# hku-mars/GS-SDF

Hardware: NVIDIA H100
Metric: train_steps_per_s (higher is better)
Workload: dtype f32

## Files before the change

gs-sdf_b200/csrc/sdf_tc.cu:

```cuda
#include "sdf_grid.cuh"
#include "sdf_loss.cuh"

namespace gssdf {

constexpr int kFwdTcThreads = 256;
constexpr int kBwdTcThreads = 512;
constexpr int kLevels = 16;
static_assert(128 * kLevels == 4 * kBwdTcThreads, "encode batches assume 4 tasks per thread");
constexpr uint32_t kWImg = 24576;
constexpr uint32_t kGW = 3072;
constexpr uint32_t kGA = 2048;
constexpr uint32_t kGA0 = 1024;
constexpr uint32_t kGL = 1024;

__device__ __forceinline__ uint32_t off_act(int r, int k, int part) {
    return (uint32_t)((r >> 3) * kGA + part * 1024 + (k >> 3) * 128 + (r & 7) * 16 + (k & 7) * 2);
}
__device__ __forceinline__ uint32_t off_feat(int r, int k, int part) {
    return (uint32_t)((r >> 3) * kGA0 + part * 512 + (k >> 3) * 128 + (r & 7) * 16 + (k & 7) * 2);
}
__device__ __forceinline__ uint32_t off_lo(int r, int k) { return (uint32_t)((r >> 3) * kGL + (k >> 3) * 128 + (r & 7) * 16 + (k & 7) * 2); }
__device__ __host__ __forceinline__ uint32_t off_w(int o, int k, int part) {
    return (uint32_t)((o >> 3) * kGW + part * 1024 + (k >> 3) * 128 + (o & 7) * 16 + (k & 7) * 2);
}

__device__ __forceinline__ uint64_t make_desc(uint32_t saddr, uint32_t lbo, uint32_t sbo) {
    uint64_t d = 0;
    d |= (uint64_t)((saddr & 0x3FFFF) >> 4);
    d |= (uint64_t)(lbo >> 4) << 16;
    d |= (uint64_t)(sbo >> 4) << 32;
    return d;
}
__device__ __forceinline__ void wg_fence() { asm volatile("wgmma.fence.sync.aligned;" ::: "memory"); }
__device__ __forceinline__ void wg_commit() { asm volatile("wgmma.commit_group.sync.aligned;" ::: "memory"); }
__device__ __forceinline__ void wg_wait() { asm volatile("wgmma.wait_group.sync.aligned 0;" ::: "memory"); }
template <int R>
__device__ __forceinline__ void acc_fence(float (&d)[R]) {
#pragma unroll
    for (int i = 0; i < R; ++i) asm volatile("" : "+f"(d[i])::"memory");
}
template <int TA, int TB>
__device__ __forceinline__ void wgmma_bf16(float (&d)[16], uint64_t a, uint64_t b, uint32_t accumulate) {
    asm volatile(
        "{\n"
        ".reg .pred p;\n"
        "setp.ne.b32 p, %18, 0;\n"
        "wgmma.mma_async.sync.aligned.m64n32k16.f32.bf16.bf16 {%0, %1, %2, %3, %4, %5, %6, %7, %8, %9, %10, %11, %12, %13, %14, %15}, "
        "%16, %17, p, 1, 1, %19, %20;\n"
        "}\n"
        : "+f"(d[0]), "+f"(d[1]), "+f"(d[2]), "+f"(d[3]), "+f"(d[4]), "+f"(d[5]), "+f"(d[6]), "+f"(d[7]), "+f"(d[8]), "+f"(d[9]),
          "+f"(d[10]), "+f"(d[11]), "+f"(d[12]), "+f"(d[13]), "+f"(d[14]), "+f"(d[15])
        : "l"(a), "l"(b), "r"(accumulate), "n"(TA), "n"(TB)
        : "memory");
}
template <int TA, int TB>
__device__ __forceinline__ void wgmma_bf16(float (&d)[32], uint64_t a, uint64_t b, uint32_t accumulate) {
    asm volatile(
        "{\n"
        ".reg .pred p;\n"
        "setp.ne.b32 p, %34, 0;\n"
        "wgmma.mma_async.sync.aligned.m64n64k16.f32.bf16.bf16 {%0, %1, %2, %3, %4, %5, %6, %7, %8, %9, %10, %11, %12, %13, %14, %15, "
        "%16, %17, %18, %19, %20, %21, %22, %23, %24, %25, %26, %27, %28, %29, %30, %31}, %32, %33, p, 1, 1, %35, %36;\n"
        "}\n"
        : "+f"(d[0]), "+f"(d[1]), "+f"(d[2]), "+f"(d[3]), "+f"(d[4]), "+f"(d[5]), "+f"(d[6]), "+f"(d[7]), "+f"(d[8]), "+f"(d[9]),
          "+f"(d[10]), "+f"(d[11]), "+f"(d[12]), "+f"(d[13]), "+f"(d[14]), "+f"(d[15]), "+f"(d[16]), "+f"(d[17]), "+f"(d[18]),
          "+f"(d[19]), "+f"(d[20]), "+f"(d[21]), "+f"(d[22]), "+f"(d[23]), "+f"(d[24]), "+f"(d[25]), "+f"(d[26]), "+f"(d[27]),
          "+f"(d[28]), "+f"(d[29]), "+f"(d[30]), "+f"(d[31])
        : "l"(a), "l"(b), "r"(accumulate), "n"(TA), "n"(TB)
        : "memory");
}
__device__ __forceinline__ bool mbar_wait_bounded(uint64_t *bar, uint32_t parity) {
    for (int it = 0; it < (1 << 24); ++it) {
        uint32_t ok;
        asm volatile(
            "{\n"
            ".reg .pred p;\n"
            "mbarrier.try_wait.parity.shared::cta.b64 p, [%1], %2;\n"
            "selp.u32 %0, 1, 0, p;\n"
            "}\n"
            : "=r"(ok)
            : "r"(smem_u32(bar)), "r"(parity)
            : "memory");
        if (ok) return true;
    }
    return false;
}

__device__ __forceinline__ void split2(float x, __nv_bfloat16 &hi, __nv_bfloat16 &mid) {
    hi = __float2bfloat16_rn(x);
    mid = __float2bfloat16_rn(x - __bfloat162float(hi));
}
__device__ __forceinline__ void split3(float x, __nv_bfloat16 &hi, __nv_bfloat16 &mid, __nv_bfloat16 &lo) {
    hi = __float2bfloat16_rn(x);
    const float r1 = x - __bfloat162float(hi);
    mid = __float2bfloat16_rn(r1);
    lo = __float2bfloat16_rn(r1 - __bfloat162float(mid));
}
__device__ __forceinline__ void store8(unsigned char *buf, unsigned char *lo_buf, int r, int k0, const float *x) {
    __nv_bfloat16 hi[8], mid[8], lo[8];
#pragma unroll
    for (int e = 0; e < 8; ++e) split3(x[e], hi[e], mid[e], lo[e]);
    *reinterpret_cast<uint4 *>(buf + off_act(r, k0, 0)) = *reinterpret_cast<uint4 *>(hi);
    *reinterpret_cast<uint4 *>(buf + off_act(r, k0, 1)) = *reinterpret_cast<uint4 *>(mid);
    if (lo_buf) *reinterpret_cast<uint4 *>(lo_buf + off_lo(r, k0)) = *reinterpret_cast<uint4 *>(lo);
}
__device__ __forceinline__ void load8_hi(const unsigned char *buf, int r, int k0, float *x) {
    const uint4 h = *reinterpret_cast<const uint4 *>(buf + off_act(r, k0, 0));
    const __nv_bfloat16 *hp = reinterpret_cast<const __nv_bfloat16 *>(&h);
#pragma unroll
    for (int e = 0; e < 8; ++e) x[e] = __bfloat162float(hp[e]);
}
__device__ __forceinline__ void load8_sum(const unsigned char *buf, int r, int k0, float *x) {
    const uint4 h = *reinterpret_cast<const uint4 *>(buf + off_act(r, k0, 0));
    const uint4 m = *reinterpret_cast<const uint4 *>(buf + off_act(r, k0, 1));
    const __nv_bfloat16 *hp = reinterpret_cast<const __nv_bfloat16 *>(&h), *mp = reinterpret_cast<const __nv_bfloat16 *>(&m);
#pragma unroll
    for (int e = 0; e < 8; ++e) x[e] = __bfloat162float(hp[e]) + __bfloat162float(mp[e]);
}
__device__ __forceinline__ void store2(unsigned char *buf, unsigned char *lo_buf, int r, int k0, float x0, float x1) {
    __nv_bfloat16 h0, m0, l0, h1, m1, l1;
    split3(x0, h0, m0, l0);
    split3(x1, h1, m1, l1);
    *reinterpret_cast<__nv_bfloat162 *>(buf + off_act(r, k0, 0)) = __halves2bfloat162(h0, h1);
    *reinterpret_cast<__nv_bfloat162 *>(buf + off_act(r, k0, 1)) = __halves2bfloat162(m0, m1);
    if (lo_buf) *reinterpret_cast<__nv_bfloat162 *>(lo_buf + off_lo(r, k0)) = __halves2bfloat162(l0, l1);
}
__device__ __forceinline__ float2 load2_hi(const unsigned char *buf, int r, int k0) {
    return __bfloat1622float2(*reinterpret_cast<const __nv_bfloat162 *>(buf + off_act(r, k0, 0)));
}
__device__ __forceinline__ float quad_sum(float v) {
    v += __shfl_xor_sync(0xffffffffu, v, 1);
    return v + __shfl_xor_sync(0xffffffffu, v, 2);
}
__device__ __forceinline__ float colsum16(float c[16], int lane) {
#pragma unroll
    for (int s = 8; s >= 1; s >>= 1) {
        const bool up = lane & s;
#pragma unroll
        for (int k = 0; k < s; ++k) {
            const float send = up ? c[k] : c[k + s], keep = up ? c[k + s] : c[k];
            c[k] = keep + __shfl_xor_sync(0xffffffffu, send, s);
        }
    }
    return c[0] + __shfl_xor_sync(0xffffffffu, c[0], 16);
}

template <bool FEAT, bool THREE, int R>
__device__ __forceinline__ void issue_layer(float (&d)[R], uint32_t a_base, uint32_t lo_base, uint32_t w_base) {
    constexpr uint32_t ga = FEAT ? kGA0 : kGA, am = FEAT ? 512u : 1024u;
    wg_fence();
#pragma unroll
    for (int ks = 0; ks < (FEAT ? kFeat : 64) / 16; ++ks) {
        const uint32_t ko = ks * 256;
        const uint64_t ah = make_desc(a_base + ko, 128, ga), amd = make_desc(a_base + am + ko, 128, ga);
        const uint64_t wh = make_desc(w_base + ko, 128, kGW), wm = make_desc(w_base + 1024 + ko, 128, kGW);
        wgmma_bf16<0, 0>(d, ah, wh, ks > 0 ? 1u : 0u);
        wgmma_bf16<0, 0>(d, ah, wm, 1);
        wgmma_bf16<0, 0>(d, amd, wh, 1);
        wgmma_bf16<0, 0>(d, amd, wm, 1);
        if constexpr (THREE) {
            wgmma_bf16<0, 0>(d, ah, make_desc(w_base + 2048 + ko, 128, kGW), 1);
            if constexpr (!FEAT) wgmma_bf16<0, 0>(d, make_desc(lo_base + ko, 128, kGL), wh, 1);
        }
    }
    wg_commit();
}
template <bool THREE = true, int R>
__device__ __forceinline__ void issue_forward_layer(float (&d)[R], int l, uint32_t a_base, uint32_t lo_base, uint32_t w_base) {
    if (l == 0) issue_layer<true, THREE>(d, a_base, lo_base, w_base);
    else issue_layer<false, THREE>(d, a_base, lo_base, w_base);
}

__global__ void __launch_bounds__(256) mlp_pack_kernel(const float *__restrict__ mlp, unsigned char *__restrict__ packed, int n_layers) {
    const int l = blockIdx.x;
    const int K = l == 0 ? kFeat : 64;
    const float *W = mlp;
    for (int q = 0; q < l; ++q) W += (size_t)64 * (q == 0 ? kFeat : 64) + 64;
    unsigned char *img = packed + (size_t)l * kWImg;
    for (int e = threadIdx.x; e < 64 * 64; e += blockDim.x) {
        const int o = e >> 6, k = e & 63;
        __nv_bfloat16 hi, mid, lo;
        split3(k < K ? __ldg(W + (size_t)o * K + k) : 0.f, hi, mid, lo);
        *reinterpret_cast<__nv_bfloat16 *>(img + off_w(o, k, 0)) = hi;
        *reinterpret_cast<__nv_bfloat16 *>(img + off_w(o, k, 1)) = mid;
        *reinterpret_cast<__nv_bfloat16 *>(img + off_w(o, k, 2)) = lo;
    }
    (void)n_layers;
}

__global__ void __launch_bounds__(kFwdTcThreads)
sdf_fwd_tc_kernel(const gssdf_sdf_fwd_args a, const GridGeom g, int64_t n_tiles) {
    constexpr int TM = 128, HID = 64;
    extern __shared__ __align__(128) unsigned char s_tc[];
    unsigned char *sA = s_tc;
    unsigned char *sF = sA + 16 * kGA;
    unsigned char *sL = sF + 16 * kGA0;
    unsigned char *sW = sL + 16 * kGL;
    float *s_bias = reinterpret_cast<float *>(sW + kWImg);
    float *s_wout = s_bias + 5 * 64;
    __shared__ __align__(8) uint64_t s_wbar;

    const int tid = threadIdx.x, warp = tid >> 5, lane = tid & 31;
    const int wg = warp >> 2, fr = 64 * wg + 16 * (warp & 3) + (lane >> 2), fc = 2 * (lane & 3);
    const int nh = 1 + a.net.n_hidden;
    const int64_t n_eval = a.n * max(a.n_variants, 1);
    const int64_t n_live = a.n_live ? min((int64_t)*a.n_live, a.n) : a.n;
    const __half2 *table = reinterpret_cast<const __half2 *>(a.net.table_half);
    const unsigned char *wimg = reinterpret_cast<const unsigned char *>(a.net.mlp_packed);

    if (tid == 0) {
        mbar_init(&s_wbar, 1);
        fence_mbar_init();
    }
    {
        const float *W = a.net.mlp;
        for (int l = 0; l < nh; ++l) {
            const int K = l == 0 ? kFeat : HID;
            if (tid < HID) s_bias[l * 64 + tid] = __ldg(W + (size_t)HID * K + tid);
            W += (size_t)HID * K + HID;
        }
        for (int e = tid; e < 2 * HID + 2; e += kFwdTcThreads) s_wout[e] = __ldg(W + e);
    }
    __syncthreads();
    bool ok = true;
    uint32_t done_layers = 0;
    for (int64_t tile = blockIdx.x; tile < n_tiles && ok; tile += gridDim.x) {
    const int64_t base = tile * TM;
    if (base % a.n >= n_live && base % a.n + TM <= a.n) continue;
    if (a.skip_base_variant && base + TM <= a.n) continue;
    const int tm = (int)min((int64_t)TM, n_eval - base);
    if (tid == 0) {
        mbar_arrive_expect_tx(&s_wbar, kWImg);
        bulk_g2s(sW, wimg, kWImg, &s_wbar);
    }
    for (int t0 = 0; t0 < TM * kLevels; t0 += 4 * kFwdTcThreads) {
        float2 f[4];
#pragma unroll
        for (int i = 0; i < 4; ++i) {
            const int task = t0 + i * kFwdTcThreads + tid, p = task % TM, lvl = task / TM;
            float x[3];
            load_x(a.net, a.x, min(base + p, n_eval - 1), a.n, a.delta, x);
            f[i] = encode_level(table, g, lvl, x);
        }
#pragma unroll
        for (int i = 0; i < 4; ++i) {
            const int task = t0 + i * kFwdTcThreads + tid, p = task % TM, lvl = task / TM;
            const bool live = p < tm && (base + p) % a.n < n_live;
            if (!live) f[i] = make_float2(0.f, 0.f);
            if (live && a.feat) *reinterpret_cast<float2 *>(a.feat + (base + p) * kFeat + 2 * lvl) = f[i];
            __nv_bfloat16 h0, m0, h1, m1;
            split2(f[i].x, h0, m0);
            split2(f[i].y, h1, m1);
            *reinterpret_cast<__nv_bfloat162 *>(sF + off_feat(p, 2 * lvl, 0)) = __halves2bfloat162(h0, h1);
            *reinterpret_cast<__nv_bfloat162 *>(sF + off_feat(p, 2 * lvl, 1)) = __halves2bfloat162(m0, m1);
        }
    }
    for (int l = 0; l < nh; ++l) {
        fence_proxy_async();
        ok = __syncthreads_and(mbar_wait_bounded(&s_wbar, (done_layers + (uint32_t)l) & 1u));
        if (!ok) break;
        float d[32];
        issue_forward_layer(d, l, smem_u32(l == 0 ? sF + 8 * wg * kGA0 : sA + 8 * wg * kGA), smem_u32(sL + 8 * wg * kGL), smem_u32(sW));
        wg_wait();
        acc_fence(d);
        __syncthreads();
        if (tid == 0 && l + 1 < nh) {
            mbar_arrive_expect_tx(&s_wbar, kWImg);
            bulk_g2s(sW, wimg + (size_t)(l + 1) * kWImg, kWImg, &s_wbar);
        }
        float act[32];
#pragma unroll
        for (int e = 0; e < 32; ++e) act[e] = fmaxf(d[e] + s_bias[l * 64 + 8 * (e >> 2) + fc + (e & 1)], 0.f);
        if (l < nh - 1) {
#pragma unroll
            for (int e = 0; e < 32; e += 2) store2(sA, sL, fr + 8 * ((e >> 1) & 1), 8 * (e >> 2) + fc, act[e], act[e + 1]);
        } else {
            float p0[2] = {0.f, 0.f}, p1[2] = {0.f, 0.f};
#pragma unroll
            for (int e = 0; e < 32; ++e) {
                const int i = (e >> 1) & 1, c = 8 * (e >> 2) + fc + (e & 1);
                p0[i] = fmaf(act[e], s_wout[c], p0[i]);
                p1[i] = fmaf(act[e], s_wout[HID + c], p1[i]);
            }
#pragma unroll
            for (int i = 0; i < 2; ++i) {
                const float s0 = quad_sum(p0[i]), s1 = quad_sum(p1[i]);
                const int p = fr + 8 * i;
                if ((lane & 3) == 0 && p < tm && (base + p) % a.n < n_live) {
                    a.sdf[base + p] = s0 + s_wout[2 * HID];
                    if (a.y1) a.y1[base + p] = s1 + s_wout[2 * HID + 1];
                }
            }
        }
    }
    done_layers += (uint32_t)nh;
    __syncthreads();
    }
    if (!ok) __trap();
}

constexpr size_t kBwdTcMain = 16 * kGA0 + 3 * 16 * kGA + 16 * kGA + 16 * kGL + kWImg;
constexpr size_t kBwdTcMisc = sizeof(float) * (4 * 64 + 132 + 384 + 4 * 128);
constexpr size_t kBwdTcMiscAnalytic = 128 * 16 * sizeof(uint16_t) + 128 * 3 * sizeof(float) + 64;
constexpr size_t bwd_tc_smem(bool analytic) { return kBwdTcMain + kBwdTcMisc + (analytic ? kBwdTcMiscAnalytic : 0); }
static_assert(bwd_tc_smem(true) + 1024 + 128 <= 196 * 1024, "the analytic variant must fit the 196 KiB shared-memory carve-out");

struct TcLossArgs {
    const float *gt_sdf, *weights, *visibilities;
    SdfLossCfg cfg;
    float *loss_out;
    int analytic;
    float align_weight;
    const float *sdf_variants;
    const uint8_t *valid_mask;
    const int32_t *n_gate;
};

template <bool FUSED, bool ANALYTIC>
__global__ void __launch_bounds__(kBwdTcThreads, 1)
sdf_bwd_tc_kernel(const gssdf_sdf_bwd_args a, const TcLossArgs lo, const GridGeom g, int64_t n_tiles) {
    constexpr int TM = 128, HID = 64, NT = kBwdTcThreads;
    extern __shared__ __align__(128) unsigned char s_tc[];
    unsigned char *sF = s_tc;
    unsigned char *sAct = sF + 16 * kGA0;
    unsigned char *sG = sAct + 3 * 16 * kGA;
    unsigned char *sL = sG + 16 * kGA;
    unsigned char *sW = sL + 16 * kGL;
    float *s_bias = reinterpret_cast<float *>(sW + kWImg);
    float *s_wout = s_bias + 4 * 64;
    float *s_dx = s_wout + 132;
    float *s_seed = s_dx;
    float *s_col = s_dx + 384;
    uint16_t *s_mask16 = reinterpret_cast<uint16_t *>(s_col + 4 * 128);
    float *s_gnum = s_col + 4 * 128 + 1024;
    int64_t *s_tbase = reinterpret_cast<int64_t *>(s_gnum + 384);
    __shared__ __align__(8) uint64_t s_wbar;

    const int tid = threadIdx.x, warp = tid >> 5, lane = tid & 31;
    const int q = warp & 3, cq = warp >> 2, row = 32 * q + lane, col0 = 16 * cq;
    const int wg = warp >> 2, fr = 16 * (warp & 3) + (lane >> 2), fc = 2 * (lane & 3);
    const int dr = 64 * (wg & 1) + fr, dc = 32 * (wg >> 1) + fc;
    const int nh = 1 + a.net.n_hidden;
    const int64_t n_eval = a.n * max(a.n_variants, 1);
    const int64_t n_live = a.n_live ? min((int64_t)*a.n_live, a.n) : a.n;
    const __half2 *table = reinterpret_cast<const __half2 *>(a.net.table_half);
    const unsigned char *wimg = reinterpret_cast<const unsigned char *>(a.net.mlp_packed);
    const int V = max(a.n_variants, 1), PT = FUSED ? TM / V : TM;
    float loss_acc = 0.f;
    constexpr bool analytic = ANALYTIC;
    static_assert(FUSED || !ANALYTIC, "the analytic eikonal path is part of the fused train kernel");
    float acc2_wo = 0.f;
    int n_coll = 0;

    if (tid == 0) {
        mbar_init(&s_wbar, 1);
        fence_mbar_init();
    }
    {
        const float *W = a.net.mlp;
        for (int l = 0; l < nh; ++l) {
            const int K = l == 0 ? kFeat : HID;
            if (tid < HID) s_bias[l * 64 + tid] = __ldg(W + (size_t)HID * K + tid);
            W += (size_t)HID * K + HID;
        }
        for (int e = tid; e < 2 * HID + 2; e += NT) s_wout[e] = __ldg(W + e);
    }
    __syncthreads();
    uint32_t ph_w = 0;
    bool ok = true, first_tile = true;
    float dbias[4] = {0.f, 0.f, 0.f, 0.f};
    float dwo0 = 0.f, dwo1 = 0.f, dbo = 0.f;
    float accW[32];
#pragma unroll
    for (int e = 0; e < 32; ++e) accW[e] = 0.f;
    float dD[16];

    auto sync_w = [&](bool wait) {
        fence_proxy_async();
        bool landed = true;
        if (wait) { landed = mbar_wait_bounded(&s_wbar, ph_w); ph_w ^= 1; }
        ok = __syncthreads_and(landed) && ok;
    };
    auto load_w = [&](int l) {
        mbar_arrive_expect_tx(&s_wbar, kWImg);
        bulk_g2s(sW, wimg + (size_t)l * kWImg, kWImg, &s_wbar);
    };
    auto finish = [&]() {
        wg_wait();
        acc_fence(dD);
        __syncthreads();
    };
    auto issue_gw = [&]() {
        const uint32_t gB = smem_u32(sG) + 8 * (wg & 1) * kGA, wB = smem_u32(sW) + 4 * (wg >> 1) * 128;
        wg_fence();
#pragma unroll
        for (int ks = 0; ks < HID / 16; ++ks) {
            const uint64_t gh = make_desc(gB + ks * 256, 128, kGA), gm = make_desc(gB + 1024 + ks * 256, 128, kGA);
            const uint64_t wh = make_desc(wB + ks * 2 * kGW, kGW, 128), wm = make_desc(wB + 1024 + ks * 2 * kGW, kGW, 128);
            wgmma_bf16<0, 1>(dD, gh, wh, ks > 0 ? 1u : 0u);
            wgmma_bf16<0, 1>(dD, gh, wm, 1);
            wgmma_bf16<0, 1>(dD, gm, wh, 1);
            wgmma_bf16<0, 1>(dD, gm, wm, 1);
        }
        wg_commit();
    };
    auto issue_dw = [&](int l) {
        if (wg != l) return;
        const uint32_t aB = smem_u32(l == 0 ? sF : sAct + (l - 1) * 16 * kGA), ga = l == 0 ? kGA0 : kGA, am = l == 0 ? 512u : 1024u;
        const uint32_t gB = smem_u32(sG);
        wg_fence();
#pragma unroll
        for (int ks = 0; ks < TM / 16; ++ks) {
            const uint64_t ah = make_desc(aB + ks * 2 * ga, ga, 128), amd = make_desc(aB + am + ks * 2 * ga, ga, 128);
            const uint64_t gh = make_desc(gB + ks * 2 * kGA, kGA, 128), gm = make_desc(gB + 1024 + ks * 2 * kGA, kGA, 128);
            wgmma_bf16<1, 1>(accW, ah, gh, 1);
            wgmma_bf16<1, 1>(accW, ah, gm, 1);
            wgmma_bf16<1, 1>(accW, amd, gh, 1);
            wgmma_bf16<1, 1>(accW, amd, gm, 1);
        }
        wg_commit();
    };


    auto second_order = [&]() {
        const int nc = n_coll;
        float *gf = reinterpret_cast<float *>(sL);
        float *s_cc = s_col;
        const float isz = a.net.inv_size != 0.f ? a.net.inv_size : 1.f;
        __syncthreads();
        for (int e = tid; e < (TM - nc) * 16; e += NT) s_mask16[nc * 16 + e] = 0;
        for (int e = tid; e < TM * 3; e += NT) s_dx[e] = 0.f;
        __syncthreads();
        auto seed_u = [&]() {
            const uint32_t bits = s_mask16[(row * 4 + nh - 1) * 4 + cq];
            float u[16];
#pragma unroll
            for (int j = 0; j < 16; ++j) u[j] = ((bits >> j) & 1u) ? s_wout[col0 + j] : 0.f;
            store8(sG, nullptr, row, col0, u);
            store8(sG, nullptr, row, col0 + 8, u + 8);
        };
        auto mask_bit = [&](int slot, int l, int e) -> bool {
            const int j = e >> 2;
            return (s_mask16[(slot * 4 + l - 1) * 4 + 2 * (wg >> 1) + (j >> 1)] >> (8 * (j & 1) + fc + (e & 1))) & 1u;
        };
        auto mask_store = [&](int l, unsigned char *dst) {
#pragma unroll
            for (int e = 0; e < 16; e += 2) {
                const int r = dr + 8 * ((e >> 1) & 1);
                store2(dst, nullptr, r, dc + 8 * (e >> 2), mask_bit(r, l, e) ? dD[e] : 0.f, mask_bit(r, l, e + 1) ? dD[e + 1] : 0.f);
            }
        };
        auto store_gf = [&]() {
            if (wg >> 1) return;
#pragma unroll
            for (int e = 0; e < 16; ++e) gf[(dr + 8 * ((e >> 1) & 1)) * 33 + dc + 8 * (e >> 2) + (e & 1)] = dD[e];
        };
        seed_u();
        if (tid == 0) { fence_proxy_async(); load_w(nh - 1); }
        for (int l = nh - 1; l >= 0 && ok; --l) {
            sync_w(true);
            if (!ok) return;
            issue_gw();
            finish();
            if (tid == 0 && l > 0) load_w(l - 1);
            if (l > 0) mask_store(l, sG);
            else store_gf();
        }
        __syncthreads();
        {
            static_assert(NT % TM == 0, "thread -> point mapping of the analytic pass");
            const int c = tid % TM;
            if (c < nc) {
                float x[3], acc[3] = {0.f, 0.f, 0.f};
                load_x(a.net, a.x, s_tbase[c / PT] + c % PT, a.n, a.delta, x);
#pragma unroll 1
                for (int lvl = tid / TM; lvl < kLevels; lvl += NT / TM) {
                    float dx[3] = {0.f, 0.f, 0.f};
                    encode_level_bwd(table, nullptr, g, lvl, x, gf[c * 33 + 2 * lvl], gf[c * 33 + 2 * lvl + 1], true, dx);
                    acc[0] += dx[0]; acc[1] += dx[1]; acc[2] += dx[2];
                }
                atomicAdd(&s_dx[c * 3 + 0], acc[0]);
                atomicAdd(&s_dx[c * 3 + 1], acc[1]);
                atomicAdd(&s_dx[c * 3 + 2], acc[2]);
            }
        }
        __syncthreads();
        if (tid < TM) {
            float cc[3] = {0.f, 0.f, 0.f};
            const SdfGate gate = tid < nc ? sdf_gate(lo.n_gate, lo.valid_mask, lo.visibilities, lo.cfg.visible_thr, s_tbase[tid / PT] + tid % PT)
                                          : SdfGate{false, true, 1.f};
            if (tid < nc && (!gate.gated || gate.gate)) {
                const float gx = s_dx[tid * 3] * isz, gy = s_dx[tid * 3 + 1] * isz, gz = s_dx[tid * 3 + 2] * isz;
                const float nl = gate.gated ? gate.ng : (float)n_live;
                const float nrm = sqrtf(gx * gx + gy * gy + gz * gz);
                const float we = lo.cfg.eikonal_weight / nl;
                loss_acc += we * (nrm - 1.f) * (nrm - 1.f);
                const float ke = nrm > 0.f ? 2.f * (nrm - 1.f) / nrm * we : 0.f;
                cc[0] = ke * gx; cc[1] = ke * gy; cc[2] = ke * gz;
                if (lo.align_weight > 0.f && (V == 7 || lo.sdf_variants)) {
                    const float wa = lo.align_weight / (3.f * nl);
                    const float *gn = s_gnum + tid * 3;
                    const float d0 = gx - gn[0], d1 = gy - gn[1], d2 = gz - gn[2];
                    loss_acc += wa * (fabsf(d0) + fabsf(d1) + fabsf(d2));
                    cc[0] += d0 > 0.f ? wa : (d0 < 0.f ? -wa : 0.f);
                    cc[1] += d1 > 0.f ? wa : (d1 < 0.f ? -wa : 0.f);
                    cc[2] += d2 > 0.f ? wa : (d2 < 0.f ? -wa : 0.f);
                }
            }
            s_cc[tid * 3] = cc[0] * isz; s_cc[tid * 3 + 1] = cc[1] * isz; s_cc[tid * 3 + 2] = cc[2] * isz;
        }
        __syncthreads();
#pragma unroll 1
        for (int task = tid; task < TM * kLevels; task += NT) {
            const int c = task % TM, lvl = task / TM;
            float r[2] = {0.f, 0.f};
            if (c < nc) {
                float x[3];
                load_x(a.net, a.x, s_tbase[c / PT] + c % PT, a.n, a.delta, x);
                encode_level_bwd2(table, a.table_grad, g, lvl, x, gf[c * 33 + 2 * lvl], gf[c * 33 + 2 * lvl + 1], s_cc + c * 3, r);
            }
            __nv_bfloat16 h0, m0, h1, m1;
            split2(r[0], h0, m0);
            split2(r[1], h1, m1);
            *reinterpret_cast<__nv_bfloat162 *>(sF + off_feat(c, 2 * lvl, 0)) = __halves2bfloat162(h0, h1);
            *reinterpret_cast<__nv_bfloat162 *>(sF + off_feat(c, 2 * lvl, 1)) = __halves2bfloat162(m0, m1);
        }
        if (!a.mlp_grad) { __syncthreads(); return; }
        __syncthreads();
        if (tid == 0) { fence_proxy_async(); load_w(0); }
        for (int l = 0; l < nh; ++l) {
            sync_w(true);
            if (!ok) return;
            issue_forward_layer<false>(dD, l, smem_u32(l == 0 ? sF + 8 * (wg & 1) * kGA0 : sAct + (l - 1) * 16 * kGA + 8 * (wg & 1) * kGA),
                                       0u, smem_u32(sW) + 4 * (wg >> 1) * kGW);
            finish();
            if (tid == 0 && (l + 1 < nh || nh > 1)) load_w(l + 1 < nh ? l + 1 : nh - 1);
            if (l < nh - 1) {
                mask_store(l + 1, sAct + l * 16 * kGA);
            } else {
#pragma unroll
                for (int e = 0; e < 16; e += 4) {
#pragma unroll
                    for (int c = 0; c < 2; ++c) {
                        float s = (mask_bit(dr, nh, e + c) ? dD[e + c] : 0.f) + (mask_bit(dr + 8, nh, e + 2 + c) ? dD[e + 2 + c] : 0.f);
                        s += __shfl_xor_sync(0xffffffffu, s, 4);
                        s += __shfl_xor_sync(0xffffffffu, s, 8);
                        s += __shfl_xor_sync(0xffffffffu, s, 16);
                        if (lane < 4) s_col[(4 * (wg & 1) + (warp & 3)) * 64 + dc + 2 * e + c] = s;
                    }
                }
            }
        }
        __syncthreads();
        if (q == 0 && lane < 16) {
            const int c = col0 + lane;
#pragma unroll
            for (int rg = 0; rg < 8; ++rg) acc2_wo += s_col[rg * 64 + c];
        }
        seed_u();
        for (int l = nh - 1; l >= 0 && ok; --l) {
            sync_w(l > 0);
            if (!ok) return;
            issue_dw(l);
            if (l > 0) issue_gw();
            finish();
            if (tid == 0 && l > 1) load_w(l - 1);
            if (l > 0) mask_store(l, sG);
        }
        __syncthreads();
    };

    for (int64_t tile = blockIdx.x; tile < n_tiles && ok; tile += gridDim.x) {
        const int64_t base = FUSED ? tile * PT : tile * TM;
        const int tm = (int)min((int64_t)TM, n_eval - base);
        if (FUSED ? base >= n_live : (base % a.n >= n_live && base % a.n + TM <= a.n)) continue;
        auto row_gi = [&](int p) -> int64_t {
            if (!FUSED) return min(base + p, n_eval - 1);
            const int j = p / V, v = p - j * V;
            return (int64_t)v * a.n + min(base + j, a.n - 1);
        };
        auto row_live = [&](int p) -> bool {
            if (!FUSED) return p < tm && (base + p) % a.n < n_live;
            const int j = p / V;
            return j < PT && base + j < n_live;
        };
        auto row_is_base = [&](int p) -> bool { return FUSED ? (p % V) == 0 : base + p < a.n; };
#define LIVE_TC(p_) row_live(p_)
        __syncthreads();
        if (tid == 0) {
            fence_proxy_async();
            load_w(0);
        }
        {
            float2 f[4];
#pragma unroll
            for (int i = 0; i < 4; ++i) {
                const int task = i * NT + tid, p = task % TM, lvl = task / TM;
                float x[3];
                load_x(a.net, a.x, row_gi(p), a.n, a.delta, x);
                f[i] = encode_level(table, g, lvl, x);
            }
#pragma unroll
            for (int i = 0; i < 4; ++i) {
                const int task = i * NT + tid, p = task % TM, lvl = task / TM;
                if (!LIVE_TC(p)) f[i] = make_float2(0.f, 0.f);
                __nv_bfloat16 h0, m0, h1, m1;
                split2(f[i].x, h0, m0);
                split2(f[i].y, h1, m1);
                *reinterpret_cast<__nv_bfloat162 *>(sF + off_feat(p, 2 * lvl, 0)) = __halves2bfloat162(h0, h1);
                *reinterpret_cast<__nv_bfloat162 *>(sF + off_feat(p, 2 * lvl, 1)) = __halves2bfloat162(m0, m1);
            }
        }
        if (!FUSED && tid < TM) {
            const bool lv = LIVE_TC(tid);
            s_seed[2 * tid] = lv ? __ldg(a.v_sdf + base + tid) : 0.f;
            s_seed[2 * tid + 1] = (lv && a.v_y1) ? __ldg(a.v_y1 + base + tid) : 0.f;
        }
        for (int l = 0; l < nh; ++l) {
            sync_w(true);
            if (!ok) break;
            issue_forward_layer(dD, l, smem_u32(l == 0 ? sF + 8 * (wg & 1) * kGA0 : sAct + (l - 1) * 16 * kGA + 8 * (wg & 1) * kGA),
                                smem_u32(sL + 8 * (wg & 1) * kGL), smem_u32(sW) + 4 * (wg >> 1) * kGW);
            finish();
            if (tid == 0 && l + 1 < nh) load_w(l + 1);
            float act[16];
#pragma unroll
            for (int e = 0; e < 16; ++e) act[e] = fmaxf(dD[e] + s_bias[l * 64 + dc + 8 * (e >> 2) + (e & 1)], 0.f);
            unsigned char *dst = (l < nh - 1) ? sAct + l * 16 * kGA : sG;
#pragma unroll
            for (int e = 0; e < 16; e += 2) store2(dst, l < nh - 1 ? sL : nullptr, dr + 8 * ((e >> 1) & 1), dc + 8 * (e >> 2), act[e], act[e + 1]);
            if (analytic) {
#pragma unroll
                for (int i = 0; i < 2; ++i) {
                    uint32_t bits[2] = {0u, 0u};
#pragma unroll
                    for (int j = 0; j < 4; ++j)
#pragma unroll
                        for (int c = 0; c < 2; ++c) bits[j >> 1] |= (act[4 * j + 2 * i + c] > 0.f ? 1u : 0u) << (8 * (j & 1) + fc + c);
#pragma unroll
                    for (int h = 0; h < 2; ++h) {
                        bits[h] |= __shfl_xor_sync(0xffffffffu, bits[h], 1);
                        bits[h] |= __shfl_xor_sync(0xffffffffu, bits[h], 2);
                    }
                    const int r = dr + 8 * i, jb = r / V;
                    if ((lane & 3) == 0 && r - jb * V == 0 && jb < PT && base + jb < n_live) {
                        s_mask16[((n_coll + jb) * 4 + l) * 4 + 2 * (wg >> 1)] = (uint16_t)bits[0];
                        s_mask16[((n_coll + jb) * 4 + l) * 4 + 2 * (wg >> 1) + 1] = (uint16_t)bits[1];
                    }
                }
            }
            if (FUSED && l == nh - 1) {
                float p0[2] = {0.f, 0.f}, p1[2] = {0.f, 0.f};
#pragma unroll
                for (int e = 0; e < 16; ++e) {
                    const int i = (e >> 1) & 1, c = dc + 8 * (e >> 2) + (e & 1);
                    p0[i] = fmaf(act[e], s_wout[c], p0[i]);
                    p1[i] = fmaf(act[e], s_wout[HID + c], p1[i]);
                }
                float *s_part = reinterpret_cast<float *>(sL);
#pragma unroll
                for (int i = 0; i < 2; ++i) {
                    const float s0 = quad_sum(p0[i]), s1 = quad_sum(p1[i]);
                    if ((lane & 3) == 0) {
                        s_part[((wg >> 1) * TM + dr + 8 * i) * 2] = s0;
                        s_part[((wg >> 1) * TM + dr + 8 * i) * 2 + 1] = s1;
                    }
                }
            }
        }
        if (!ok) break;
        __syncthreads();
        if (FUSED) {
            float *s_part = reinterpret_cast<float *>(sL), *s_out = s_part + 2 * TM * 2;
            if (tid < TM) {
                s_out[2 * tid] = s_part[tid * 2] + s_part[(TM + tid) * 2] + s_wout[2 * HID];
                s_out[2 * tid + 1] = s_part[tid * 2 + 1] + s_part[(TM + tid) * 2 + 1] + s_wout[2 * HID + 1];
                s_seed[2 * tid] = 0.f;
                s_seed[2 * tid + 1] = 0.f;
            }
            __syncthreads();
            if (tid < PT && base + tid < n_live) {
                const int64_t i = base + tid;
                float sv[7], v_s[7], v_y;
                for (int v = 0; v < V; ++v) sv[v] = s_out[2 * (tid * V + v)];
                SdfLossCfg cfg1 = lo.cfg;
                if (analytic) {
                    cfg1.eikonal_weight = 0.f;
                    if (tid == 0) s_tbase[n_coll / PT] = base;
                    if (V == 1 && lo.sdf_variants) {
                        for (int v = 1; v < 7; ++v) sv[v] = __ldg(lo.sdf_variants + (int64_t)v * a.n + i);
                    }
                    if (V == 7 || lo.sdf_variants) {
                        const float inv2d = 0.5f / lo.cfg.delta;
                        s_gnum[(n_coll + tid) * 3 + 0] = (sv[1] - sv[2]) * inv2d;
                        s_gnum[(n_coll + tid) * 3 + 1] = (sv[3] - sv[4]) * inv2d;
                        s_gnum[(n_coll + tid) * 3 + 2] = (sv[5] - sv[6]) * inv2d;
                    }
                }
                loss_acc += sdf_point_loss(cfg1, (float)n_live, V, sv, s_out[2 * tid * V + 1], lo.gt_sdf != nullptr,
                                           lo.gt_sdf ? __ldg(lo.gt_sdf + i) : 0.f, lo.weights != nullptr, lo.weights ? __ldg(lo.weights + i) : 0.f,
                                           lo.visibilities != nullptr, lo.visibilities ? __ldg(lo.visibilities + i) : 0.f, v_s, v_y,
                                           sdf_gate(lo.n_gate, lo.valid_mask, lo.visibilities, lo.cfg.visible_thr, i));
                for (int v = 0; v < V; ++v) s_seed[2 * (tid * V + v)] = v_s[v];
                s_seed[2 * tid * V + 1] = v_y;
            }
            __syncthreads();
        }
        {
            float an[16], gl[16];
            load8_sum(sG, row, col0, an);
            load8_sum(sG, row, col0 + 8, an + 8);
            const float v0 = s_seed[2 * row], v1 = s_seed[2 * row + 1];
#pragma unroll
            for (int j = 0; j < 16; ++j) gl[j] = an[j] > 0.f ? v0 * s_wout[col0 + j] + v1 * s_wout[HID + col0 + j] : 0.f;
            store8(sG, nullptr, row, col0, gl);
            store8(sG, nullptr, row, col0 + 8, gl + 8);
            if (a.mlp_grad) {
                float c0[16], c1[16];
#pragma unroll
                for (int j = 0; j < 16; ++j) { c0[j] = v0 * an[j]; c1[j] = v1 * an[j]; }
                const float s0 = colsum16(c0, lane), s1 = colsum16(c1, lane);
                if (lane < 16) {
                    s_col[q * 128 + col0 + lane] = s0;
                    s_col[q * 128 + 64 + col0 + lane] = s1;
                }
                if (cq == 0) {
                    const float b0 = warp_sum(v0), b1 = warp_sum(v1);
                    if (lane == 0) { s_dx[256 + 2 * q] = b0; s_dx[256 + 2 * q + 1] = b1; }
                }
            }
        }
        __syncthreads();
        if (a.mlp_grad) {
            if (tid < 2 * HID) {
                const float s = s_col[tid] + s_col[128 + tid] + s_col[256 + tid] + s_col[384 + tid];
                if (tid < HID) dwo0 += s; else dwo1 += s;
            } else if (tid < 2 * HID + 2) {
                const int o = tid - 2 * HID;
                dbo += s_dx[256 + o] + s_dx[258 + o] + s_dx[260 + o] + s_dx[262 + o];
            }
        }
        for (int l = nh - 1; l >= 0; --l) {
            sync_w(l < nh - 1);
            if (!ok) break;
            if (a.mlp_grad) issue_dw(l);
            issue_gw();
            if (a.mlp_grad) {
                float c[16];
                load8_sum(sG, row, col0, c);
                load8_sum(sG, row, col0 + 8, c + 8);
                const float s = colsum16(c, lane);
                if (lane < 16) s_col[q * 128 + col0 + lane] = s;
            }
            finish();
            if (tid == 0 && l > 0) load_w(l - 1);
            if (l > 0) {
#pragma unroll
                for (int e = 0; e < 16; e += 2) {
                    const int r = dr + 8 * ((e >> 1) & 1), c = dc + 8 * (e >> 2);
                    const float2 m = load2_hi(sAct + (l - 1) * 16 * kGA, r, c);
                    store2(sG, nullptr, r, c, m.x > 0.f ? dD[e] : 0.f, m.y > 0.f ? dD[e + 1] : 0.f);
                }
            } else if ((wg >> 1) == 0) {
                float *gf = reinterpret_cast<float *>(sL);
#pragma unroll
                for (int e = 0; e < 16; ++e) gf[(dr + 8 * ((e >> 1) & 1)) * 33 + dc + 8 * (e >> 2) + (e & 1)] = dD[e];
            }
            __syncthreads();
            if (a.mlp_grad && q == 0 && lane < 16) {
                const int c = col0 + lane;
                dbias[l] += s_col[c] + s_col[128 + c] + s_col[256 + c] + s_col[384 + c];
            }
        }
        if (!ok) break;
        for (int e = tid; e < TM * 3; e += NT) s_dx[e] = 0.f;
        __syncthreads();
        {
            const float *gf = reinterpret_cast<const float *>(sL);
            for (int task = tid; task < TM * g.L; task += NT) {
                const int p = task % TM, lvl = task / TM;
                if (LIVE_TC(p)) {
                    float x[3], dx[3] = {0.f, 0.f, 0.f};
                    load_x(a.net, a.x, row_gi(p), a.n, a.delta, x);
                    const bool want_dx = a.v_x != nullptr && row_is_base(p);
                    encode_level_bwd(table, a.table_grad, g, lvl, x, gf[p * 33 + 2 * lvl], gf[p * 33 + 2 * lvl + 1], want_dx, dx);
                    if (want_dx) {
                        atomicAdd(&s_dx[p * 3 + 0], dx[0]);
                        atomicAdd(&s_dx[p * 3 + 1], dx[1]);
                        atomicAdd(&s_dx[p * 3 + 2], dx[2]);
                    }
                }
            }
        }
        __syncthreads();
        if (a.v_x) {
            const float sc = a.net.inv_size != 0.f ? a.net.inv_size : 1.f;
            if (FUSED) {
                for (int e = tid; e < PT * 3; e += NT) {
                    const int j = e / 3, d = e - 3 * j;
                    if (base + j < n_live) a.v_x[(base + j) * 3 + d] = s_dx[(j * V) * 3 + d] * sc;
                }
            } else {
                for (int e = tid; e < tm * 3; e += NT)
                    if (base + e / 3 < n_live) a.v_x[base * 3 + e] = s_dx[e] * sc;
            }
        }
        first_tile = false;
        if (ANALYTIC) {
            n_coll += (int)min((int64_t)PT, n_live - base);
            if (n_coll + PT > TM) {
                second_order();
                n_coll = 0;
                if (!ok) break;
            }
        }

#undef LIVE_TC
    }
    if (ANALYTIC && ok && n_coll > 0) second_order();
    __syncthreads();
    if (ok && a.mlp_grad && !first_tile) {
        float *G = a.mlp_grad;
        for (int l = 0; l < nh; ++l) {
            const int K = l == 0 ? kFeat : HID;
            if (wg == l) {
#pragma unroll
                for (int e = 0; e < 32; ++e) {
                    const int k = fr + 8 * ((e >> 1) & 1), o = 8 * (e >> 2) + fc + (e & 1);
                    if (k < K) atomicAdd(G + (size_t)o * K + k, accW[e]);
                }
            }
            if (q == 0 && lane < 16) atomicAdd(G + (size_t)HID * K + col0 + lane, dbias[l]);
            G += (size_t)HID * K + HID;
        }
        if (ANALYTIC && q == 0 && lane < 16) atomicAdd(G + col0 + lane, acc2_wo);
        if (tid < HID) atomicAdd(G + tid, dwo0);
        else if (tid < 2 * HID) atomicAdd(G + tid, dwo1);
        else if (tid < 2 * HID + 2) atomicAdd(G + tid, dbo);
    }
    if (FUSED && lo.loss_out) {
        loss_acc = warp_sum(loss_acc);
        if (lane == 0 && loss_acc != 0.f) atomicAdd(lo.loss_out, loss_acc);
    }
    if (!ok) __trap();
}

}

using namespace gssdf;

extern "C" int64_t gssdf_sdf_mlp_packed_bytes(const gssdf_sdf_net *net) {
    if (!net || net->hidden_dim != 64 || net->n_hidden < 0 || net->n_hidden > 3) return -1;
    return (int64_t)(1 + net->n_hidden) * kWImg;
}

extern "C" int gssdf_sdf_mlp_pack(const gssdf_sdf_net *net, void *packed, gssdf_stream_t stream) {
    GSSDF_REQUIRE(net && packed, GSSDF_EINVAL, "sdf_mlp_pack: null argument");
    GSSDF_REQUIRE(net->hidden_dim == 64 && net->n_levels * net->n_features_per_level == kFeat, GSSDF_EUNSUPPORTED,
                  "sdf_mlp_pack: the tensor-core decoder needs hidden_dim 64 and 32 encoded features");
    GSSDF_REQUIRE(net->n_hidden >= 0 && net->n_hidden <= 3, GSSDF_EUNSUPPORTED, "sdf_mlp_pack: n_hidden %d not in [0,3]", net->n_hidden);
    GSSDF_REQUIRE(net->mlp, GSSDF_EINVAL, "sdf_mlp_pack: net.mlp is null");
    GSSDF_REQUIRE(((uintptr_t)packed & 15) == 0, GSSDF_EINVAL, "sdf_mlp_pack: packed must be 16-byte aligned");
    mlp_pack_kernel<<<1 + net->n_hidden, 256, 0, (cudaStream_t)stream>>>(net->mlp, reinterpret_cast<unsigned char *>(packed), 1 + net->n_hidden);
    GSSDF_LAUNCH_OK("mlp_pack_kernel");
    return GSSDF_OK;
}

static int check_tc(const char *who, const gssdf_sdf_net &net) {
    GSSDF_REQUIRE(net.hidden_dim == 64, GSSDF_EUNSUPPORTED, "%s: the tensor-core decoder needs hidden_dim 64", who);
    GSSDF_REQUIRE(net.n_hidden <= 3, GSSDF_EUNSUPPORTED, "%s: the tensor-core decoder supports n_hidden <= 3 (one weight-gradient accumulator per warpgroup)", who);
    GSSDF_REQUIRE(net.mlp_packed && ((uintptr_t)net.mlp_packed & 15) == 0, GSSDF_EINVAL,
                  "%s: mlp_mode 1 needs net.mlp_packed (gssdf_sdf_mlp_pack), 16-byte aligned", who);
    return GSSDF_OK;
}

extern "C" int gssdf_sdf_fwd_tc_launch(const gssdf_sdf_fwd_args *a, const gssdf::GridGeom *g, gssdf_stream_t stream) {
    int rc = check_tc("sdf_fwd", a->net);
    if (rc) return rc;
    const size_t smem = 16 * kGA + 16 * kGA0 + 16 * kGL + kWImg + sizeof(float) * (5 * 64 + 132) + 1024;
    static bool attr_set = false;
    if (!attr_set) {
        GSSDF_CUDA_OK(cudaFuncSetAttribute(sdf_fwd_tc_kernel, cudaFuncAttributeMaxDynamicSharedMemorySize, (int)smem));
        attr_set = true;
    }
    const int64_t n_tiles = (a->n * (a->n_variants > 1 ? a->n_variants : 1) + 127) / 128;
    int dev = 0, sms = 132;
    cudaGetDevice(&dev);
    cudaDeviceGetAttribute(&sms, cudaDevAttrMultiProcessorCount, dev);
    const int grid = (int)std::min<int64_t>(n_tiles, (int64_t)2 * sms);
    sdf_fwd_tc_kernel<<<grid, kFwdTcThreads, smem, (cudaStream_t)stream>>>(*a, *g, n_tiles);
    GSSDF_LAUNCH_OK("sdf_fwd_tc_kernel");
    return GSSDF_OK;
}

extern "C" int gssdf_sdf_bwd_tc_launch(const gssdf_sdf_bwd_args *a, const gssdf::GridGeom *g, gssdf_stream_t stream) {
    int rc = check_tc("sdf_bwd", a->net);
    if (rc) return rc;
    GSSDF_CUDA_OK(cudaFuncSetAttribute(sdf_bwd_tc_kernel<false, false>, cudaFuncAttributeMaxDynamicSharedMemorySize, (int)bwd_tc_smem(false)));
    const int64_t n_tiles = (a->n * (a->n_variants > 1 ? a->n_variants : 1) + 127) / 128;
    int dev = 0, sms = 132;
    cudaGetDevice(&dev);
    cudaDeviceGetAttribute(&sms, cudaDevAttrMultiProcessorCount, dev);
    const int grid = (int)std::min<int64_t>(n_tiles, (int64_t)sms);
    sdf_bwd_tc_kernel<false, false><<<grid, kBwdTcThreads, bwd_tc_smem(false), (cudaStream_t)stream>>>(*a, TcLossArgs{}, *g, n_tiles);
    GSSDF_LAUNCH_OK("sdf_bwd_tc_kernel");
    return GSSDF_OK;
}

extern "C" int gssdf_sdf_train(const gssdf_sdf_train_args *t, gssdf_stream_t stream) {
    GSSDF_REQUIRE(t != nullptr, GSSDF_EINVAL, "sdf_train: null args");
    GSSDF_REQUIRE(t->net.mlp_mode == 1, GSSDF_EUNSUPPORTED, "sdf_train: the fused forward+loss+backward kernel exists for mlp_mode 1 only "
                  "(use gssdf_sdf_fwd + gssdf_sdf_loss + gssdf_sdf_bwd otherwise)");
    GSSDF_REQUIRE(t->net.n_levels == 16 && t->net.n_features_per_level == 2, GSSDF_EUNSUPPORTED, "sdf_train: 16 levels x 2 features only");
    int rc = check_tc("sdf_train", t->net);
    if (rc) return rc;
    GSSDF_REQUIRE(t->n >= 0, GSSDF_EINVAL, "sdf_train: negative n");
    if (t->n == 0) return GSSDF_OK;
    GSSDF_REQUIRE(t->x && t->net.table_half && t->net.mlp, GSSDF_EINVAL, "sdf_train: x, table_half, mlp must be non-null");
    GSSDF_REQUIRE(t->n_variants == 1 || t->n_variants == 7, GSSDF_EINVAL, "sdf_train: n_variants must be 1 or 7");
    GSSDF_REQUIRE(t->n_variants == 1 || t->delta > 0.f, GSSDF_EINVAL, "sdf_train: delta must be positive");
    GSSDF_REQUIRE(((uintptr_t)t->table_grad & 7) == 0, GSSDF_EINVAL, "sdf_train: table_grad must be 8-byte aligned");
    gssdf_sdf_bwd_args a{};
    a.net = t->net; a.n = t->n; a.x = t->x; a.n_variants = t->n_variants; a.delta = t->delta; a.n_live = t->n_live;
    a.table_grad = t->table_grad; a.mlp_grad = t->mlp_grad; a.v_x = t->v_x;
    TcLossArgs lo{t->gt_sdf, t->weights, t->visibilities,
                  SdfLossCfg{t->bce_isigma, t->bce_weight, t->eikonal_weight, t->gs_sdf_weight, t->delta, t->visible_thr}, t->loss_out,
                  t->eikonal_mode, t->align_weight, t->n_variants == 1 ? t->sdf_variants : nullptr, t->valid_mask, t->n_gate};
    GSSDF_REQUIRE(t->eikonal_mode == 0 || t->eikonal_mode == 1, GSSDF_EINVAL, "sdf_train: eikonal_mode must be 0 or 1");
    GSSDF_REQUIRE(!(t->eikonal_mode == 1 && t->align_weight > 0.f) || t->n_variants == 7 || t->sdf_variants, GSSDF_EINVAL,
                  "sdf_train: the align loss needs the numerical gradient: n_variants 7 or sdf_variants");
    GSSDF_REQUIRE(!t->sdf_variants || t->delta > 0.f, GSSDF_EINVAL, "sdf_train: sdf_variants needs the delta they were evaluated with");
    GSSDF_REQUIRE(t->eikonal_mode == 1 || t->align_weight == 0.f, GSSDF_EINVAL, "sdf_train: align_weight needs eikonal_mode 1");
    const GridGeom g = make_grid(t->net);
    GSSDF_CUDA_OK(cudaFuncSetAttribute(sdf_bwd_tc_kernel<true, false>, cudaFuncAttributeMaxDynamicSharedMemorySize, (int)bwd_tc_smem(false)));
    GSSDF_CUDA_OK(cudaFuncSetAttribute(sdf_bwd_tc_kernel<true, true>, cudaFuncAttributeMaxDynamicSharedMemorySize, (int)bwd_tc_smem(true)));
    const int pt = 128 / t->n_variants;
    const int64_t n_tiles = (t->n + pt - 1) / pt;
    int dev = 0, sms = 132;
    cudaGetDevice(&dev);
    cudaDeviceGetAttribute(&sms, cudaDevAttrMultiProcessorCount, dev);
    const int grid = (int)std::min<int64_t>(n_tiles, (int64_t)sms);
    if (t->eikonal_mode == 1)
        sdf_bwd_tc_kernel<true, true><<<grid, kBwdTcThreads, bwd_tc_smem(true), (cudaStream_t)stream>>>(a, lo, g, n_tiles);
    else
        sdf_bwd_tc_kernel<true, false><<<grid, kBwdTcThreads, bwd_tc_smem(false), (cudaStream_t)stream>>>(a, lo, g, n_tiles);
    GSSDF_LAUNCH_OK("sdf_train_kernel");
    return GSSDF_OK;
}
```

Measured before the change: 175.8.

## Enumerate live tiles directly, park weight-grad accumulators in smem, reorder colsum

The forward kernel now counts only the tiles that hold live rows in each variant and maps the block-strided index onto them, instead of striding over every tile and skipping dead ones. The backward kernel moves its 32 per-thread weight-gradient accumulators into shared memory (reusing the activation buffer) while the encoding phases run, and restores them around the MLP phases, to cut register pressure. The column-sum scratch now reuses one array, and the colsum work is issued before the async dW/gW MMAs rather than after. These changes add smem traffic and a per-tile variant-walk loop, and parking in sAct relies on that buffer being free during the parked phases.

```diff
diff --git a/gs-sdf_b200/csrc/sdf_tc.cu b/gs-sdf_b200/csrc/sdf_tc.cu
--- a/gs-sdf_b200/csrc/sdf_tc.cu
+++ b/gs-sdf_b200/csrc/sdf_tc.cu
@@ -224,10 +224,29 @@
     __syncthreads();
     bool ok = true;
     uint32_t done_layers = 0;
-    for (int64_t tile = blockIdx.x; tile < n_tiles && ok; tile += gridDim.x) {
+    const int nv = max(a.n_variants, 1);
+    auto live_tiles = [&](int v, int64_t &first) -> int64_t {
+        if (n_live <= 0) return 0;
+        first = (int64_t)v * a.n / TM;
+        if (v == 0 && a.skip_base_variant) first = a.n / TM;
+        if (v > 0) first = max(first, ((int64_t)(v - 1) * a.n + n_live - 1) / TM + 1);
+        return max(((int64_t)v * a.n + n_live - 1) / TM - first + 1, (int64_t)0);
+    };
+    int64_t n_live_tiles = 0;
+    for (int v = 0; v < nv; ++v) {
+        int64_t f;
+        n_live_tiles += live_tiles(v, f);
+    }
+    (void)n_tiles;
+    for (int64_t k = blockIdx.x; k < n_live_tiles && ok; k += gridDim.x) {
+    int64_t tile = 0, r = k;
+    for (int v = 0; v < nv; ++v) {
+        int64_t f;
+        const int64_t c = live_tiles(v, f);
+        if (r < c) { tile = f + r; break; }
+        r -= c;
+    }
     const int64_t base = tile * TM;
-    if (base % a.n >= n_live && base % a.n + TM <= a.n) continue;
-    if (a.skip_base_variant && base + TM <= a.n) continue;
     const int tm = (int)min((int64_t)TM, n_eval - base);
     if (tid == 0) {
         mbar_arrive_expect_tx(&s_wbar, kWImg);
@@ -371,8 +390,18 @@
     float dbias[4] = {0.f, 0.f, 0.f, 0.f};
     float dwo0 = 0.f, dwo1 = 0.f, dbo = 0.f;
     float accW[32];
+    float *s_park = reinterpret_cast<float *>(sAct);
+    auto park_w = [&]() {
+#pragma unroll
+        for (int e = 0; e < 32; ++e) s_park[e * NT + tid] = accW[e];
+    };
+    auto unpark_w = [&]() {
+#pragma unroll
+        for (int e = 0; e < 32; ++e) accW[e] = s_park[e * NT + tid];
+    };
 #pragma unroll
     for (int e = 0; e < 32; ++e) accW[e] = 0.f;
+    park_w();
     float dD[16];
 
     auto sync_w = [&](bool wait) {
@@ -526,6 +555,7 @@
             *reinterpret_cast<__nv_bfloat162 *>(sF + off_feat(c, 2 * lvl, 1)) = __halves2bfloat162(m0, m1);
         }
         if (!a.mlp_grad) { __syncthreads(); return; }
+        unpark_w();
         __syncthreads();
         if (tid == 0) { fence_proxy_async(); load_w(0); }
         for (int l = 0; l < nh; ++l) {
@@ -568,6 +598,7 @@
             if (l > 0) mask_store(l, sG);
         }
         __syncthreads();
+        park_w();
     };
 
     for (int64_t tile = blockIdx.x; tile < n_tiles && ok; tile += gridDim.x) {
@@ -616,6 +647,7 @@
             s_seed[2 * tid] = lv ? __ldg(a.v_sdf + base + tid) : 0.f;
             s_seed[2 * tid + 1] = (lv && a.v_y1) ? __ldg(a.v_y1 + base + tid) : 0.f;
         }
+        unpark_w();
         for (int l = 0; l < nh; ++l) {
             sync_w(true);
             if (!ok) break;
@@ -716,10 +748,13 @@
             store8(sG, nullptr, row, col0, gl);
             store8(sG, nullptr, row, col0 + 8, gl + 8);
             if (a.mlp_grad) {
-                float c0[16], c1[16];
-#pragma unroll
-                for (int j = 0; j < 16; ++j) { c0[j] = v0 * an[j]; c1[j] = v1 * an[j]; }
-                const float s0 = colsum16(c0, lane), s1 = colsum16(c1, lane);
+                float c[16];
+#pragma unroll
+                for (int j = 0; j < 16; ++j) c[j] = v0 * an[j];
+                const float s0 = colsum16(c, lane);
+#pragma unroll
+                for (int j = 0; j < 16; ++j) c[j] = v1 * an[j];
+                const float s1 = colsum16(c, lane);
                 if (lane < 16) {
                     s_col[q * 128 + col0 + lane] = s0;
                     s_col[q * 128 + 64 + col0 + lane] = s1;
@@ -743,8 +778,6 @@
         for (int l = nh - 1; l >= 0; --l) {
             sync_w(l < nh - 1);
             if (!ok) break;
-            if (a.mlp_grad) issue_dw(l);
-            issue_gw();
             if (a.mlp_grad) {
                 float c[16];
                 load8_sum(sG, row, col0, c);
@@ -752,6 +785,8 @@
                 const float s = colsum16(c, lane);
                 if (lane < 16) s_col[q * 128 + col0 + lane] = s;
             }
+            if (a.mlp_grad) issue_dw(l);
+            issue_gw();
             finish();
             if (tid == 0 && l > 0) load_w(l - 1);
             if (l > 0) {
@@ -773,6 +808,7 @@
             }
         }
         if (!ok) break;
+        park_w();
         for (int e = tid; e < TM * 3; e += NT) s_dx[e] = 0.f;
         __syncthreads();
         {
@@ -820,6 +856,7 @@
     if (ANALYTIC && ok && n_coll > 0) second_order();
     __syncthreads();
     if (ok && a.mlp_grad && !first_tile) {
+        unpark_w();
         float *G = a.mlp_grad;
         for (int l = 0; l < nh; ++l) {
             const int K = l == 0 ? kFeat : HID;
```

Result: faster. 179.2 (median of 6 runs) (+2.0%).
